# clvrai/mopa-rl

Hardware: AMD Instinct MI355X
Metric: valid-state collision checks/sec (higher is better)
Workload: dtype f64; 1 GPU; SawyerPushObstacle-v0 state validity (FK + collision), 4096 envs/GPU x 256 states/env per step, states 50% uniform joint-box samples + 50% near-init N(0,0.3); envs_per_gpu=4096, states_per_env=256, parallelism=env-shard x1

## Files before the change

include/mopa_hip.h:

```cpp
#ifndef MOPA_HIP_H
#define MOPA_HIP_H
#include <stdint.h>

#ifdef __cplusplus
extern "C" {
#endif

#define MOPA_OK 0
#define MOPA_ERR_INVALID_ARG 1
#define MOPA_ERR_UNSUPPORTED 2
#define MOPA_ERR_HIP 3
#define MOPA_ERR_LIMIT 4

#define MOPA_PLAN_OK 0
#define MOPA_PLAN_NO_EXACT (-4)
#define MOPA_PLAN_INVALID_GOAL (-5)

#define MOPA_FAR 1.0e10

enum { MOPA_GEOM_PLANE = 0, MOPA_GEOM_SPHERE = 2, MOPA_GEOM_CAPSULE = 3, MOPA_GEOM_CYLINDER = 5, MOPA_GEOM_BOX = 6, MOPA_GEOM_MESH = 7 };
enum { MOPA_JNT_FREE = 0, MOPA_JNT_BALL = 1, MOPA_JNT_SLIDE = 2, MOPA_JNT_HINGE = 3 };

typedef struct MopaModel {
    int32_t nq, nbody, njnt, ngeom, npair;
// ... 70 lines not shown
int mopa_glue_rows_batch(MopaScene *scene, double *path_dev , const int32_t *path_len_dev ,
                         const double *attached_dev , int64_t E, int32_t max_path, void *stream);
int mopa_scene_num_active(const MopaScene *scene);
int mopa_scene_active_idx(const MopaScene *scene, int32_t *out );
int mopa_scene_num_pairs(const MopaScene *scene);
int mopa_scene_lds_bytes(const MopaScene *scene);
int mopa_scene_valid_kernel(const MopaScene *scene, int64_t N, char *out, int32_t cap );
int mopa_scene_motion_kernel(const MopaScene *scene, int64_t N, char *out, int32_t cap );
int mopa_scene_k1_baked(const MopaScene *scene);
int mopa_scene_k1_export(const MopaSceneDesc *desc, int64_t *sizes , double *dbl, int32_t *ints, int32_t *tab, void *hdr,
                         uint64_t *fingerprint);
int mopa_scene_hdr_offset(const char *field);
int mopa_scene_k1_export_glued(const MopaSceneDesc *desc, int32_t body_a, int32_t body_b, int64_t *sizes , double *dbl, int32_t *ints,
                               int32_t *tab, void *hdr, uint64_t *fingerprint);
int mopa_k1_baked_fk_host(int index, int64_t n, const double *q_active, const double *qpos_env, double *out);

int mopa_is_valid_batch(MopaScene *scene, const double *q_active_dev , const double *qpos_env_dev ,
                        int64_t N, int64_t samples_per_env, uint8_t *valid_dev , double *min_dist_dev ,
                        void *stream);

int mopa_check_motion_batch(MopaScene *scene, const double *qa_dev , const double *qb_dev ,
                            const double *qpos_env_dev , int64_t N, int64_t samples_per_env,
                            uint8_t *valid_dev , void *stream);

int mopa_plan_batch(MopaScene *scene, const double *start_dev , const double *goal_dev , int64_t E,
                    const MopaPlanParams *params, double *path_dev , int32_t *path_len_dev ,
                    int32_t *status_dev , int64_t *n_checks_dev , void *stream);

int mopa_simplify_paths_batch(MopaScene *scene, int64_t E, int32_t max_path, double *path_dev ,
                              int32_t *path_len_dev , const int32_t *status_dev , uint64_t seed,
                              uint64_t env_id_base, const uint64_t *env_ids_dev , const uint64_t *seeds_dev ,
                              int32_t passes, int64_t *info_dev , void *stream);
int mopa_simplify_paths_max_path(const MopaScene *scene);

// ... 388 lines not shown
```

mopa_rl_amd/_lib.py:

```python
from __future__ import annotations

import ctypes as C
import os
from typing import Optional

import numpy as np

_HERE = os.path.dirname(os.path.abspath(__file__))
LIB_PATH = os.environ.get("MOPA_HIP_LIB", os.path.join(_HERE, "csrc", "libmopa_hip.so"))

MOPA_OK = 0
MOPA_FAR = 1.0e10
PLAN_OK, PLAN_NO_EXACT, PLAN_INVALID_GOAL = 0, -4, -5

_dp = C.POINTER(C.c_double)
_ip = C.POINTER(C.c_int32)

EXPORTED_SYMBOLS = [
    "mopa_last_error", "mopa_version", "mopa_device_count", "mopa_scene_create", "mopa_scene_destroy",
    "mopa_scene_create_glued", "mopa_scene_glue", "mopa_glue_attach_batch", "mopa_glue_rows_batch", "mopa_scene_k1_export_glued",
    "mopa_scene_num_active", "mopa_scene_active_idx", "mopa_scene_num_pairs", "mopa_scene_lds_bytes", "mopa_scene_valid_kernel",
    "mopa_scene_motion_kernel",
    "mopa_scene_k1_baked", "mopa_scene_k1_export", "mopa_scene_hdr_offset", "mopa_k1_baked_fk_host",
    "mopa_is_valid_batch", "mopa_check_motion_batch", "mopa_plan_batch", "mopa_simplify_paths_batch", "mopa_simplify_paths_max_path", "mopa_shortcut_paths_batch", "mopa_shortcut_paths_max_path", "mopa_smooth_paths_batch", "mopa_smooth_paths_max_path",
    "mopa_plan_star_batch", "mopa_plan_star", "mopa_plan_star_k", "mopa_star_params_size",
    "mopa_plan_race_batch", "mopa_plan_race", "mopa_race_params_size", "mopa_pullback_batch", "mopa_is_valid_state", "mopa_plan",
    "mopa_planner_status", "mopa_debug_fk", "mopa_debug_pair_dist", "mopa_contacts_batch", "mopa_contacts_state",
    "mopa_contact_frames_batch", "mopa_contact_frames_state", "mopa_geom_frames_batch", "mopa_geom_frames_host",
    "mopa_env_create", "mopa_env_destroy", "mopa_env_obs_dim", "mopa_env_action_dim", "mopa_env_step_batch", "mopa_env_exec_batch", "mopa_env_desired_batch",
    "mopa_env_attach_dynamics", "mopa_env_attach_contacts", "mopa_env_set_contact_stats", "mopa_rollout_stage", "mopa_rollout_pool_pick", "mopa_rollout_step_size", "mopa_reuse_batch", "mopa_replay_append", "mopa_replay_sample", "mopa_ct_desc_size", "mopa_env_contact_arena", "mopa_env_dyn_dofs", "mopa_env_dyn_qvel_width", "mopa_env_dyn_forward_batch", "mopa_env_dyn_substeps_batch", "mopa_env_step_dyn_batch",
    "mopa_pusher_dyn_desc_size", "mopa_env_attach_pusher_dynamics", "mopa_env_set_pusher_stats", "mopa_env_pusher_substeps_batch",
    "mopa_env_step_pusher_batch", "mopa_env_set_contact_force",
    "mopa_ik_create", "mopa_ik_destroy", "mopa_ik_solve_batch", "mopa_ik_site_pose_batch", "mopa_ik_targets_batch",
    "mopa_ik_targets_pos_batch", "mopa_ik_displacement_pos_batch",
    "mopa_paths_unwrap_batch", "mopa_paths_unwrap_seam_batch", "mopa_paths_walk_batch", "mopa_paths_assemble_batch", "mopa_interpolate_batch",
]


class MopaError(RuntimeError):
# ... 148 lines not shown
    L.mopa_version.restype = C.c_char_p
    L.mopa_device_count.restype = C.c_int
    L.mopa_scene_create.argtypes = [C.POINTER(MopaSceneDesc), C.POINTER(vp)]
    L.mopa_scene_destroy.argtypes = [vp]
    L.mopa_scene_destroy.restype = None
    L.mopa_scene_create_glued.argtypes = [C.POINTER(MopaSceneDesc), C.c_int32, C.c_int32, C.POINTER(vp)]
    L.mopa_scene_glue.argtypes = [vp, _ip]
    L.mopa_glue_attach_batch.argtypes = [vp, vp, C.c_int64, vp, vp]
    L.mopa_glue_rows_batch.argtypes = [vp, vp, vp, vp, C.c_int64, C.c_int32, vp]
    L.mopa_scene_k1_export_glued.argtypes = [vp, C.c_int32, C.c_int32, vp, vp, vp, vp, vp, vp]
    L.mopa_scene_num_active.argtypes = [vp]
    L.mopa_scene_active_idx.argtypes = [vp, _ip]
    L.mopa_scene_num_pairs.argtypes = [vp]
    L.mopa_scene_lds_bytes.argtypes = [vp]
    L.mopa_is_valid_batch.argtypes = [vp, vp, vp, C.c_int64, C.c_int64, vp, vp, vp]
    L.mopa_check_motion_batch.argtypes = [vp, vp, vp, vp, C.c_int64, C.c_int64, vp, vp]
    L.mopa_plan_batch.argtypes = [vp, vp, vp, C.c_int64, C.POINTER(MopaPlanParams), vp, vp, vp, vp, vp]
    L.mopa_simplify_paths_batch.argtypes = [vp, C.c_int64, C.c_int32, vp, vp, vp, C.c_uint64, C.c_uint64, vp, vp, C.c_int32, vp, vp]
    L.mopa_simplify_paths_max_path.argtypes = [vp]
    L.mopa_shortcut_paths_batch.argtypes = [vp, C.c_int64, C.c_int32, vp, vp, vp, C.c_uint64, C.c_uint64, vp, vp, C.c_int32, C.c_int32, vp, vp]
    L.mopa_shortcut_paths_max_path.argtypes = [vp]
    L.mopa_smooth_paths_batch.argtypes = [vp, C.c_int64, C.c_int32, vp, vp, vp, C.c_uint64, C.c_uint64, vp, vp, C.c_int32, C.c_int32, vp, vp]
    L.mopa_smooth_paths_max_path.argtypes = [vp]
    L.mopa_plan_star_batch.argtypes = [vp, vp, vp, C.c_int64, C.POINTER(MopaStarParams), vp, vp, vp, vp, vp, vp]
    L.mopa_plan_star.argtypes = [vp, _dp, _dp, C.POINTER(MopaStarParams), _dp, C.POINTER(C.c_int32), C.POINTER(C.c_int32),
                                 C.POINTER(C.c_double), C.POINTER(C.c_int64)]
    L.mopa_plan_star_k.argtypes = [C.c_int32, C.c_int64, C.c_double]
    L.mopa_star_params_size.argtypes = []
    L.mopa_plan_race_batch.argtypes = [vp, vp, vp, C.c_int64, C.POINTER(MopaRaceParams), vp, vp, vp, vp, vp, vp, vp, vp]
    L.mopa_plan_race.argtypes = [vp, _dp, _dp, C.POINTER(MopaRaceParams), _dp, C.POINTER(C.c_int32), C.POINTER(C.c_int32),
# ... 49 lines not shown
    L.mopa_ik_destroy.argtypes = [vp]
    L.mopa_ik_destroy.restype = None
    L.mopa_ik_solve_batch.argtypes = [vp, C.c_int64, vp, vp, vp, C.c_double, C.c_int32, C.c_double, C.c_double, C.c_double, C.c_double,
                                      vp, vp, vp, vp]
    L.mopa_ik_site_pose_batch.argtypes = [vp, C.c_int64, vp, vp, vp, vp]
    L.mopa_ik_targets_batch.argtypes = [vp, C.c_int64, vp, vp, vp, C.c_int64, C.c_double, C.POINTER(C.c_double), C.POINTER(C.c_double), vp, vp, vp]
    L.mopa_ik_targets_pos_batch.argtypes = [vp, C.c_int64, vp, vp, C.c_int64, C.c_int32, C.c_double, C.POINTER(C.c_double), C.POINTER(C.c_double), vp, vp]
    L.mopa_ik_displacement_pos_batch.argtypes = [vp, C.c_int64, vp, vp, C.c_int64, C.c_int32, C.c_double, C.POINTER(C.c_double), C.POINTER(C.c_double),
                                                 C.c_int32, C.c_double, C.c_double, C.c_double, C.c_double, vp, vp, vp, vp, vp, vp, vp]
    L.mopa_scene_valid_kernel.argtypes = [vp, C.c_int64, C.c_char_p, C.c_int32]
    L.mopa_scene_motion_kernel.argtypes = [vp, C.c_int64, C.c_char_p, C.c_int32]
    L.mopa_scene_k1_baked.argtypes = [vp]
    L.mopa_scene_k1_export.argtypes = [vp, vp, vp, vp, vp, vp, vp]
    L.mopa_scene_hdr_offset.argtypes = [C.c_char_p]
    L.mopa_k1_baked_fk_host.argtypes = [C.c_int, C.c_int64, vp, vp, vp]
    i32, i64, f64 = C.c_int32, C.c_int64, C.c_double
    L.mopa_paths_unwrap_batch.argtypes = [C.c_int, i64, i32, i32, vp, i32, vp, vp, vp, f64, i32, vp, vp, vp, vp, vp, vp, vp, vp]
    L.mopa_paths_unwrap_seam_batch.argtypes = [C.c_int, i64, i32, i32, vp, i32, vp, vp, vp, f64, i32, vp, vp, vp, vp, vp, vp, vp, C.c_uint64, vp]
    L.mopa_paths_walk_batch.argtypes = [C.c_int, i64, i32, i32, vp, i32, vp, vp, f64, vp, vp, vp, vp, vp, vp, vp, vp]
    L.mopa_paths_assemble_batch.argtypes = [C.c_int, i64, i32, vp, i32, vp, vp, vp, vp, vp, vp, vp, i32, vp, vp]
    L.mopa_interpolate_batch.argtypes = [vp, i64, i32, i32, vp, vp, f64, vp, vp, vp, vp, vp]
    _lib = L
    return L


def check(rc: int) -> None:
    if rc != MOPA_OK:
        raise MopaError(f"libmopa_hip error {rc}: {lib().mopa_last_error().decode()}")


# ... 344 lines not shown
```

mopa_rl_amd/batch.py:

```python
from __future__ import annotations

import ctypes as C
import os

import numpy as np
from typing import Optional, Tuple

from . import _lib


def _torch():
    import torch
    return torch


def _ptr(t) -> C.c_void_p:
    return C.c_void_p(t.data_ptr())


def _check_f64(t, name, cols=None):
    torch = _torch()
    if t.dtype != torch.float64 or not t.is_cuda or not t.is_contiguous():
        raise _lib.MopaError(f"{name} must be a contiguous float64 tensor on the GPU")
    if cols is not None and (t.dim() != 2 or t.shape[1] != cols):
# ... 99 lines not shown
    return (4 if path_shortcut else 0) | vertex


def k9_entry(vertex_simplify, path_shortcut, path_smooth) -> Optional[str]:
    return "smooth_paths" if path_smooth else "shortcut_paths" if path_shortcut else "simplify_paths" if vertex_simplify else None


class BatchPlanner:

    def __init__(self, scene: "_lib.Scene"):
        self.scene = scene
        self.na = scene.na
        self.nq = scene.nq

    def is_valid(self, q_active, qpos_env, samples_per_env: Optional[int] = None, want_min_dist: bool = False,
                 out=None, stream=None, guard: bool = False):
        torch = _torch()
        _check_f64(q_active, "q_active", self.na)
        _check_f64(qpos_env, "qpos_env", self.nq)
        N = q_active.shape[0]
        spe = int(samples_per_env) if samples_per_env is not None else max(1, N // max(1, qpos_env.shape[0]))
        if N and (N + spe - 1) // spe > qpos_env.shape[0]:
            raise _lib.MopaError("qpos_env has fewer rows than ceil(N / samples_per_env)")
        valid = out if out is not None else torch.empty(N, dtype=torch.uint8, device=q_active.device)
        md = torch.empty(N, dtype=torch.float64, device=q_active.device) if want_min_dist else None
        _lib.check(_lib.lib().mopa_is_valid_batch(self.scene.handle, _ptr(q_active), _ptr(qpos_env), N, spe, _ptr(valid),
                                                  _ptr(md) if md is not None else None, _stream_handle(stream)))
        if guard and self.scene.npair_pruned and N:
            sc = self.scene
            dev = q_active.device
            if getattr(self, "_guard_t", None) is None or self._guard_t[0].device != dev:
                pos = {int(a): k for k, a in enumerate(sc.active_idx)}
                act = [k for k, a in enumerate(sc.guard_adr) if int(a) in pos]
                pas = [k for k, a in enumerate(sc.guard_adr) if int(a) not in pos]
                mk = lambda a, dt: torch.as_tensor(np.asarray(a), dtype=dt, device=dev)
                self._guard_t = (mk([pos[int(sc.guard_adr[k])] for k in act], torch.long), mk(sc.guard_lo[act], torch.float64), mk(sc.guard_hi[act], torch.float64),
                                 mk(sc.guard_adr[pas], torch.long), mk(sc.guard_lo[pas], torch.float64), mk(sc.guard_hi[pas], torch.float64))
            ia, la, ha, ip_, lp, hp = self._guard_t
            qa = q_active[:, ia]
            oor = ((qa < la) | (qa > ha)).any(dim=1)
# ... 348 lines not shown
```

mopa_rl_amd/csrc/mopa_hip.hip:

```cpp
#include <hip/hip_runtime.h>

#include <algorithm>
#include <cmath>
#include <cstdio>
#include <cstdlib>
#include <cstddef>
#include <cstring>
#include <string>
#include <utility>
#include <vector>

#include <map>
#include <mutex>
#include "../../include/mopa_hip.h"
#include "mopa_device.hpp"
#include "mopa_frames.hpp"
#include "mopa_fk.hpp"
#include "mopa_host.hpp"

using namespace mopa;

static thread_local std::string g_err;
int mopa_fail(int code, const std::string &msg) {
    g_err = msg;
// ... 482 lines not shown
extern "C" int mopa_scene_k1_export_glued(const MopaSceneDesc *desc, int32_t body_a, int32_t body_b, int64_t *sizes, double *dbl, int32_t *ints,
                                          int32_t *tab, void *hdr, uint64_t *fingerprint) {
    if (body_a < 0 || body_b < 0) return fail(MOPA_ERR_INVALID_ARG, "glue: body id out of range");
    return scene_k1_export(desc, body_a, body_b, sizes, dbl, ints, tab, hdr, fingerprint);
}

extern "C" int mopa_scene_hdr_offset(const char *field) {
    if (!field) return -1;
#define MOPA_HDR_FIELD(f_) if (!std::strcmp(field, #f_)) return (int)offsetof(SceneHdr, f_);
    MOPA_HDR_FIELD(na) MOPA_HDR_FIELD(nq) MOPA_HDR_FIELD(n_pq) MOPA_HDR_FIELD(nmb) MOPA_HDR_FIELD(nmg) MOPA_HDR_FIELD(nsf)
    MOPA_HDR_FIELD(n_save) MOPA_HDR_FIELD(n_pas_b) MOPA_HDR_FIELD(n_dbl) MOPA_HDR_FIELD(n_int) MOPA_HDR_FIELD(o_mbr) MOPA_HDR_FIELD(o_mbd)
    MOPA_HDR_FIELD(o_mgd) MOPA_HDR_FIELD(o_sf_pos) MOPA_HDR_FIELD(o_sf_quat) MOPA_HDR_FIELD(o_sf_mat) MOPA_HDR_FIELD(o_act_ref)
    MOPA_HDR_FIELD(o_pq_adr) MOPA_HDR_FIELD(o_mg_geom) MOPA_HDR_FIELD(thr)
    MOPA_HDR_FIELD(o_mb_parent) MOPA_HDR_FIELD(o_chain_adr) MOPA_HDR_FIELD(o_chain_len) MOPA_HDR_FIELD(o_chain_items) MOPA_HDR_FIELD(o_g_mb)
    MOPA_HDR_FIELD(o_mb_load) MOPA_HDR_FIELD(o_mb_save) MOPA_HDR_FIELD(pfk_maxlen) MOPA_HDR_FIELD(n_gp) MOPA_HDR_FIELD(npair) MOPA_HDR_FIELD(o_pairs)
#undef MOPA_HDR_FIELD
    return -1;
}

namespace {
struct K1HostSink {
    double *out;
    void operator()(int m, V3 gp, Q4 gq) {
        double *o = out + 12 * m;
        o[0] = gp.x; o[1] = gp.y; o[2] = gp.z;
        quat2mat(o + 3, gq);
    }
};
template <class TR>
void k1_fk_host(int64_t n, const double *q_active, const double *qpos_env, double *out) {
    for (int64_t s = 0; s < n; s++) {
        K1HostSink sink{out + (size_t)s * 12 * TR::nmg};
        k1_fk_baked<TR>(q_active + (size_t)s * TR::na, qpos_env + (size_t)s * TR::nq, sink, std::make_integer_sequence<int, TR::nmb>{});
    }
}
}
extern "C" int mopa_k1_baked_fk_host(int index, int64_t n, const double *q_active, const double *qpos_env, double *out) {
    if (n < 0 || (n > 0 && (!q_active || !qpos_env || !out))) return fail(MOPA_ERR_INVALID_ARG, "null argument / negative count");
#define MOPA_K1_FK_HOST(i_, T_) if (index == i_) { k1_fk_host<T_>(n, q_active, qpos_env, out); return MOPA_OK; }
    MOPA_K1_BAKED_SCENES(MOPA_K1_FK_HOST)
#undef MOPA_K1_FK_HOST
    return fail(MOPA_ERR_INVALID_ARG, "no baked scene #" + std::to_string(index));
}

static int scene_create(const MopaSceneDesc *desc, int glue_a, int glue_b, MopaScene **out) {
    if (!desc || !out) return fail(MOPA_ERR_INVALID_ARG, "null argument");
    MopaScene *S = new MopaScene();
    {
        const int rc = scene_build_host(desc, S, glue_a, glue_b);
        if (rc != MOPA_OK) { delete S; return rc; }
    }
    {
        const char *eb = std::getenv("MOPA_K1_BAKED");
        const uint64_t fp = k1_fingerprint(S);
        const bool allowed = !(eb && std::string(eb) == "0") && S->k1.use_v5 && S->k1.v5_cen_lds && S->n_mesh_gp == 0 && S->glue_b < 0;
        S->k1_baked = allowed ? k1_baked_index(fp) : 0;
// ... 186 lines not shown
```

mopa_rl_amd/csrc/mopa_valid_launch.inc:

```

static int64_t k1_lane_min(const MopaScene *S) { return S->k1.v2_forced ? 64 : std::max<int64_t>(64, (int64_t)S->n_cu * 36); }
static int64_t k1_motion_expand_min(const MopaScene *S) { return S->k1.v2_forced ? 64 : std::max<int64_t>(64, (int64_t)S->n_cu * 16); }

using K1FnV1 = decltype(&k_is_valid<false, false>);
using K1FnV2 = decltype(&k_is_valid_v2<false, false>);
using K1FnV5 = decltype(&k_is_valid_v5<false, true, false>);
#define MOPA_K1_COUNT(i_, T_) +1
constexpr int kK1BakedScenes = 0 MOPA_K1_BAKED_SCENES(MOPA_K1_COUNT);
#undef MOPA_K1_COUNT

static K1FnV1 k1_kernel_v1(bool want_md, bool mesh) {
    static const K1FnV1 tab[2][2] = {{k_is_valid<false, false>, k_is_valid<true, false>}, {k_is_valid<false, true>, k_is_valid<true, true>}};
    return tab[mesh][want_md];
}
static K1FnV2 k1_kernel_v2(bool want_md, bool mesh) {
    static const K1FnV2 tab[2][2] = {{k_is_valid_v2<false, false>, k_is_valid_v2<true, false>}, {k_is_valid_v2<false, true>, k_is_valid_v2<true, true>}};
    return tab[mesh][want_md];
}
static K1FnV5 k1_kernel_v5(bool want_md, bool cen_lds, bool gate, int baked) {
    static const K1FnV5 generic[3][2] = {{k_is_valid_v5<false, true, false>, k_is_valid_v5<true, true, false>},
                                         {k_is_valid_v5<false, false, false>, k_is_valid_v5<true, false, false>},
                                         {k_is_valid_v5<false, false, true>, k_is_valid_v5<true, false, true>}};
    if (cen_lds && gate) return nullptr;
    if (!baked) return generic[cen_lds ? 0 : (gate ? 2 : 1)][want_md];
// ... 191 lines not shown
    {
        unsigned long long hp[6];
        (void)hipStreamSynchronize(st);
        (void)hipMemcpy(hp, d_prof, 48, hipMemcpyDeviceToHost);
        if (hp[5]) fprintf(stderr, "[v2 profile] per tile cycles: body %.0f geom %.0f cull+push %.0f flush %.0f total %.0f (tiles %llu)\n",
                           (double)hp[0] / hp[5], (double)hp[1] / hp[5], (double)hp[2] / hp[5], (double)hp[3] / hp[5], (double)hp[4] / hp[5], hp[5]);
    }
#endif
    return MOPA_OK;
}

extern "C" int mopa_is_valid_batch(MopaScene *S, const double *q_active, const double *qpos_env, int64_t N,
                                   int64_t samples_per_env, uint8_t *valid, double *min_dist, void *stream) {
    return launch_is_valid(S, q_active, qpos_env, N, samples_per_env, nullptr, valid, min_dist, stream, nullptr, true);
}
```

mopa_rl_amd/csrc/mopa_valid_v5.inc:

```

constexpr int kEntCapV5Max = 1024;
constexpr int kBatCapV5 = 128;
constexpr int kMprCapV5 = 128;
constexpr int kMprRow = 32;
constexpr float kCullEps = 2.0e-5f;

struct K1Generic {
    static constexpr bool kBaked = false;
};
#include "mopa_valid_v5_baked.inc"

template <class TR, int M, bool WANT_MD, int K>
MOPA_D void v5_cull_baked(float cx, float cy, float cz, const float *cen_lane, unsigned &surv_lo, unsigned &surv_hi,
                          unsigned long long &deep_mask, unsigned long long &any_kept) {
    constexpr int e = TR::padr[M] + K;
    constexpr float c0 = __builtin_bit_cast(float, TR::tab[8 * e + 0]), c1 = __builtin_bit_cast(float, TR::tab[8 * e + 1]);
    constexpr float c2 = __builtin_bit_cast(float, TR::tab[8 * e + 2]), c3 = __builtin_bit_cast(float, TR::tab[8 * e + 3]);
    constexpr float c4 = __builtin_bit_cast(float, TR::tab[8 * e + 4]), c5 = __builtin_bit_cast(float, TR::tab[8 * e + 5]);
    constexpr float c6 = __builtin_bit_cast(float, TR::tab[8 * e + 6]);
    bool keep;
    if constexpr (K < TR::nmov[M]) {
        const float *pc = cen_lane + ((TR::tab[8 * e + 7] >> 14) & 0xff) * 3 * 64;
        const float dx = cx - pc[0], dy = cy - pc[64], dz = cz - pc[128];
        const float d2 = fmaf(dz, dz, fmaf(dy, dy, dx * dx));
        if constexpr (!WANT_MD && TR::tab[8 * e + 0] != 0u) deep_mask |= __ballot(d2 < c0);
        keep = !(d2 > c3);
    } else if constexpr (K < TR::nmov[M] + TR::nstat[M]) {
        const float dx = cx - c0, dy = cy - c1, dz = cz - c2;
        keep = !((fmaf(dz, dz, fmaf(dy, dy, dx * dx)) > c3) | (fabsf(dx) > c4) | (fabsf(dy) > c5) | (fabsf(dz) > c6));
    } else {
        const float dx = cx - c0, dy = cy - c1, dz = cz - c2;
        keep = !(fmaf(dz, c6, fmaf(dy, c5, dx * c4)) > c3);
    }
    if constexpr (K < 32) surv_lo |= keep ? (1u << K) : 0u;
    else surv_hi |= keep ? (1u << (K - 32)) : 0u;
    any_kept |= __ballot(keep) ? (1ull << K) : 0ull;
}
template <class TR, int M, bool WANT_MD, int... K>
MOPA_D void v5_pass_a_baked(float cx, float cy, float cz, const float *cen_lane, unsigned &surv_lo, unsigned &surv_hi,
                            unsigned long long &deep_mask, unsigned long long &any_kept, std::integer_sequence<int, K...>) {
    (v5_cull_baked<TR, M, WANT_MD, K>(cx, cy, cz, cen_lane, surv_lo, surv_hi, deep_mask, any_kept), ...);
}
template <class TR, bool WANT_MD, int... M>
MOPA_D void v5_pass_a_dispatch(int m, float cx, float cy, float cz, const float *cen_lane, unsigned &surv_lo, unsigned &surv_hi,
                               unsigned long long &deep_mask, unsigned long long &any_kept, std::integer_sequence<int, M...>) {
    (void)((m == M ? (v5_pass_a_baked<TR, M, WANT_MD>(cx, cy, cz, cen_lane, surv_lo, surv_hi, deep_mask, any_kept,
                                                     std::make_integer_sequence<int, TR::pnum[M]>{}), true)
                   : false) || ...);
}

MOPA_HD constexpr double k1_bits(unsigned long long b) { return __builtin_bit_cast(double, b); }
template <class TR>
struct K1FkRegs {
    V3 pos;
    Q4 quat;
    double mat[9];
    V3 save_pos[TR::n_save];
    Q4 save_quat[TR::n_save];
};
template <class TR, int M, class Sink>
MOPA_HD void k1_fk_geom(const K1FkRegs<TR> &r, Sink &sink) {
    constexpr const unsigned long long *gd = TR::fk_gd[M];
    const V3 gp = add3(r.pos, mat_vec(r.mat, V3{k1_bits(gd[0]), k1_bits(gd[1]), k1_bits(gd[2])}));
    const Q4 gq = quat_mul(r.quat, Q4{k1_bits(gd[3]), k1_bits(gd[4]), k1_bits(gd[5]), k1_bits(gd[6])});
    sink(M, gp, gq);
}
template <class TR, int B, class Sink, int... G>
MOPA_HD void k1_fk_body(K1FkRegs<TR> &r, const double *qact, const double *sn, const double *cs, const double *pv, Sink &sink,
                        std::integer_sequence<int, G...>) {
    constexpr const int *bi = TR::fk_body[B];
    constexpr int load = bi[0], sf = bi[1], save = bi[2], mgadr = bi[3], jn = bi[5], jt = bi[6], src = bi[8];
    constexpr bool jp0 = bi[7] != 0;
    constexpr const unsigned long long *bd = TR::fk_bd[B];
    static_assert(jn <= 1 && sizeof...(G) == bi[4], "baked walk: one joint per body at most");
    if constexpr (jn == 1 && jt == J_FREE) {
        fk_free_step(pv + (src - TR::na), r.pos, r.quat);
    } else {
        V3 ppos;
        Q4 pquat;
        if constexpr (load == -2) {
// ... 18 lines not shown
            if constexpr (src < TR::na) apply_joint_sc(jt, ax, jp, jp0, qact[src] - ref, sn[src], cs[src], r.pos, r.quat);
            else apply_joint(jt, ax, jp, jp0, pv[src - TR::na] - ref, r.pos, r.quat);
        }
        r.quat = quat_normalize(r.quat);
    }
    quat2mat(r.mat, r.quat);
    if constexpr (save >= 0) {
        r.save_pos[save] = r.pos;
        r.save_quat[save] = r.quat;
    }
    (k1_fk_geom<TR, mgadr + G>(r, sink), ...);
}
template <class TR, class Sink, int... B>
MOPA_HD void k1_fk_baked(const double *qa_row, const double *env_row, Sink &sink, std::integer_sequence<int, B...>) {
    static_assert(TR::na <= 8 && TR::n_pq >= 1 && TR::n_save >= 1, "baked walk: at most 8 active values; array sizes padded to 1");
    double qact[TR::na], pv[TR::n_pq], sn[TR::na], cs[TR::na];
#pragma unroll
    for (int a = 0; a < TR::na; a++) qact[a] = qa_row[a];
#pragma unroll
    for (int k = 0; k < TR::n_pq; k++) pv[k] = env_row[TR::fk_pq_adr[k]];
#pragma unroll
    for (int a = 0; a < TR::na; a++) mopa_sincos(0.5 * (qact[a] - k1_bits(TR::fk_act_ref[a])), sn[a], cs[a]);
    K1FkRegs<TR> r;
    r.pos = V3{0.0, 0.0, 0.0};
    r.quat = Q4{1.0, 0.0, 0.0, 0.0};
    (k1_fk_body<TR, B>(r, qact, sn, cs, pv, sink, std::make_integer_sequence<int, TR::fk_body[B][4]>{}), ...);
}
struct V5FkSink {
    double *slab;
    float *cen;
    MOPA_D void operator()(int m, V3 gp, Q4 gq) {
        double *sp = slab + (size_t)m * kSlabStride;
        pose7_st<64>(sp, gp, gq);
        float *cp = cen + (size_t)m * 3 * 64;
        cp[0] = (float)gp.x; cp[64] = (float)gp.y; cp[128] = (float)gp.z;
    }
};

struct V5Lds {
    float *cen;
    unsigned *ent;
    unsigned *bat;
    unsigned *bat2;
    unsigned long long *bad;
    unsigned long long *md;
    bool tp;
};
MOPA_HD int v5_lds_per_wave(int nmg, int ent_cap, bool want_md) { return ((nmg * 3 * 64 * 4) + ent_cap * 4 + 2 * kBatCapV5 * 4 + (want_md ? 64 * 8 : 0) + 8 + 15) & ~15; }

MOPA_D void v5_load_rec2(double (&R1)[15], double (&R2)[15], const SceneHdr &h, const double *D, const double *slab_tile,
                         int gA, int movA, int slotA, int gB, int movB, int slotB, int slA, int slB) {
// ... 200 lines not shown
    const long long n_tiles = (N + 63) >> 6;
    for (;;) {
        long long tile = 0;
        if (lane == 0) tile = (long long)atomicAdd(tile_ctr, 1ull);
        tile = __shfl(tile, 0, 64);
        const bool fin = tile >= n_tiles;
        if (!fin) {
        long long s = tile * 64 + lane;
        const bool act = s < N;
        if (!act) s = N - 1;
        const double *qa_row = q_active + s * h.na;
        const double *env_row = qpos_env + (env_idx ? (long long)env_idx[s] : s / samples_per_env) * h.nq;
        if (lane == 0) *q.bad = 0ull;
        if (WANT_MD) q.md[lane] = f64_sortable(0.0);

#ifdef MOPA_V5_FK_REPS
        for (int fk_rep = 0; fk_rep < MOPA_V5_FK_REPS; fk_rep++)
#endif
        if constexpr (TR::kBaked) {
            double *fk_slab = slab;
            asm volatile("" : "+v"(fk_slab));
            V5FkSink sink{fk_slab, q.cen + lane};
            k1_fk_baked<TR>(qa_row, env_row, sink, std::make_integer_sequence<int, TR::nmb>{});
#ifdef MOPA_V5_FK_REPS
            asm volatile("" ::: "memory");
#endif
        } else {
            double *ps = reinterpret_cast<double *>(q.ent);
            bool tile_poses = false;
            if (!GATE && h.n_pas_b > 0) {
                const unsigned long long er = (unsigned long long)env_row;
                const unsigned long long e0 = ((unsigned long long)(unsigned)__builtin_amdgcn_readfirstlane((int)(er >> 32)) << 32) | (unsigned)__builtin_amdgcn_readfirstlane((int)(unsigned)er);
                tile_poses = __all(er == e0);
            }
            q.tp = !GATE && tile_poses;
            if (!GATE && tile_poses) {
                for (int lv = 0; lv < h.n_pas_lv; lv++) {
                    const int i = s_int[h.o_pas_lv + lv] + lane;
// ... 153 lines not shown
                for (int m = bi.mgadr; m < bi.mgadr + bi.mgnum; m++) {
                    const double *gd = s_dbl + h.o_mgd + 8 * m;
                    const V3 gp = add3(pos, mat_vec(mat, ld3(gd)));
                    const Q4 gq = quat_mul(quat, Q4{gd[3], gd[4], gd[5], gd[6]});
                    double *sp = slab + (size_t)m * kSlabStride;
                    pose7_st<64>(sp, gp, gq);
                    float *cp = CEN_LDS ? q.cen + (size_t)m * 3 * 64 + lane : gcen + (size_t)m * 3 * 64;
                    cp[0] = (float)gp.x; cp[64] = (float)gp.y; cp[128] = (float)gp.z;
                }
            }
        }
        wave_sync();

        bool dead = !act;
        bool need_mesh = false;
        int n_ent = 0;
        unsigned present = 0u;
        for (int m = 0; m < h.nmg; m++) {
            int p0, pn;
            if (GATE) {
                p0 = g_tab[8 * h.n_gp + h.nmg + 2 * m]; pn = g_tab[8 * h.n_gp + h.nmg + 2 * m + 1];
            } else {
                const V2GeomI gi = *reinterpret_cast<const V2GeomI *>(GI + h.o_mgr + 4 * m);
                p0 = gi.padr; pn = gi.pnum;
            }
            if (pn == 0) continue;
            float cx, cy, cz;
            if (CEN_LDS) {
                const float *cp = q.cen + (size_t)m * 3 * 64 + lane;
                cx = cp[0]; cy = cp[64]; cz = cp[128];
// ... 217 lines not shown
```

mopa_rl_amd/csrc/mopa_valid_v5_baked.inc:

```

struct K1Baked_SawyerPushObstacle {
    static constexpr bool kBaked = true;
    static constexpr unsigned long long kFingerprint = 0x85dfbe79baeda04bull;
    static constexpr int nmg = 14;
    static constexpr int padr[nmg] = {0, 1, 3, 4, 5, 10, 15, 29, 47, 65, 83, 101, 119, 138};
    static constexpr int pnum[nmg] = {1, 2, 1, 1, 5, 5, 14, 18, 18, 18, 18, 18, 19, 17};
    static constexpr int nmov[nmg] = {0, 0, 0, 0, 1, 1, 3, 5, 5, 5, 5, 5, 6, 13};
    static constexpr int nstat[nmg] = {0, 1, 0, 0, 3, 3, 10, 12, 12, 12, 12, 12, 12, 3};
    static constexpr int npl[nmg] = {1, 1, 1, 1, 1, 1, 1, 1, 1, 1, 1, 1, 1, 1};
    static constexpr unsigned tab[1240] = {
        0x00000000u, 0x00000000u, 0x00000000u, 0x3d8f66a5u, 0x00000000u, 0x00000000u, 0x3f800000u, 0x40001000u,
        0x00000000u, 0x00000000u, 0x3f88f5c3u, 0x3dd74fecu, 0x3e852158u, 0x3e852158u, 0x3e999c39u, 0x00000603u,
        0x00000000u, 0x00000000u, 0x00000000u, 0x3e38572au, 0x00000000u, 0x00000000u, 0x3f800000u, 0x40001000u,
        0x00000000u, 0x00000000u, 0x00000000u, 0x3e0e4865u, 0x00000000u, 0x00000000u, 0x3f800000u, 0x40001300u,
        0x00000000u, 0x00000000u, 0x00000000u, 0x3d8f66a5u, 0x00000000u, 0x00000000u, 0x3f800000u, 0x40001000u,
        0x3d67a9acu, 0x00000000u, 0x00000000u, 0x3e2c26b4u, 0x00000000u, 0x00000000u, 0x00000000u, 0x00007505u,
        0xbea66666u, 0x00000000u, 0x3f11eb85u, 0x3eac19a5u, 0x3eae171au, 0x3edc2b95u, 0x3efd7344u, 0x00000901u,
        0xbca3d70au, 0x00000000u, 0x3f28f5c3u, 0x3eb150c3u, 0x3ed1ee24u, 0x3ed1ee24u, 0x3f0a3ec0u, 0x00000b02u,
        0x00000000u, 0x00000000u, 0x3f88f5c3u, 0x3e0f6b23u, 0x3e9ebaf1u, 0x3e9ebaf1u, 0x3eb335d2u, 0x00000b03u,
        0x00000000u, 0x00000000u, 0x00000000u, 0x3e6b8a5du, 0x00000000u, 0x00000000u, 0x3f800000u, 0x40001100u,
        0x3d5e062au, 0x00000000u, 0x00000000u, 0x3db2405bu, 0x00000000u, 0x00000000u, 0x00000000u, 0x00007505u,
        0xbea66666u, 0x00000000u, 0x3f11eb85u, 0x3e5d3203u, 0x3e666ba4u, 0x3ea14a4du, 0x3ec291fcu, 0x00000901u,
        0xbca3d70au, 0x00000000u, 0x3f28f5c3u, 0x3e65928au, 0x3e970cddu, 0x3e970cddu, 0x3ed99c39u, 0x00000b02u,
        0x00000000u, 0x00000000u, 0x3f88f5c3u, 0x3d89a388u, 0x3e47b352u, 0x3e47b352u, 0x3e70a915u, 0x00000b03u,
// ... 182 lines not shown
        {0x0000000000000000ull, 0x0000000000000000ull, 0x3fbc28f5c28f5c29ull, 0x3ff0000000000000ull, 0x0000000000000000ull, 0x0000000000000000ull, 0x0000000000000000ull},
        {0x0000000000000000ull, 0x0000000000000000ull, 0x3fa999999999999aull, 0x3ff0000000000000ull, 0x0000000000000000ull, 0x0000000000000000ull, 0x0000000000000000ull},
        {0x0000000000000000ull, 0x3f8eb851eb851eb8ull, 0xbf847ae147ae147bull, 0x3ff0000000000000ull, 0x0000000000000000ull, 0x0000000000000000ull, 0x0000000000000000ull},
        {0x0000000000000000ull, 0x0000000000000000ull, 0x0000000000000000ull, 0x3ff0000000000000ull, 0x0000000000000000ull, 0x0000000000000000ull, 0x0000000000000000ull},
        {0xbf989374bc6a7efaull, 0x0000000000000000ull, 0x0000000000000000ull, 0x3fe6a2ecb934b59aull, 0x0000000000000000ull, 0x3fe69e4fd79ac743ull, 0x0000000000000000ull},
        {0x0000000000000000ull, 0x0000000000000000ull, 0x0000000000000000ull, 0x3ff0000000000000ull, 0x0000000000000000ull, 0x0000000000000000ull, 0x0000000000000000ull},
        {0x0000000000000000ull, 0xbfa47ae147ae147bull, 0x0000000000000000ull, 0x3ff0000000000000ull, 0x0000000000000000ull, 0x0000000000000000ull, 0x0000000000000000ull},
        {0x0000000000000000ull, 0x0000000000000000ull, 0x0000000000000000ull, 0x3ff0000000000000ull, 0x0000000000000000ull, 0x0000000000000000ull, 0x0000000000000000ull},
    };
    static constexpr unsigned long long fk_sf[nsf][16] = {
        {0x0000000000000000ull, 0x0000000000000000ull, 0x0000000000000000ull, 0x3ff0000000000000ull, 0x0000000000000000ull, 0x0000000000000000ull, 0x0000000000000000ull, 0x3ff0000000000000ull, 0x0000000000000000ull, 0x0000000000000000ull, 0x0000000000000000ull, 0x3ff0000000000000ull, 0x0000000000000000ull, 0x0000000000000000ull, 0x0000000000000000ull, 0x3ff0000000000000ull},
        {0x0000000000000000ull, 0x0000000000000000ull, 0x3fee666666666666ull, 0x3ff0000000000000ull, 0x0000000000000000ull, 0x0000000000000000ull, 0x0000000000000000ull, 0x3ff0000000000000ull, 0x0000000000000000ull, 0x0000000000000000ull, 0x0000000000000000ull, 0x3ff0000000000000ull, 0x0000000000000000ull, 0x0000000000000000ull, 0x0000000000000000ull, 0x3ff0000000000000ull},
    };
    static constexpr unsigned long long fk_act_ref[na] = {0x0000000000000000ull, 0x0000000000000000ull, 0x0000000000000000ull, 0x0000000000000000ull, 0x0000000000000000ull, 0x0000000000000000ull, 0x0000000000000000ull};
    static constexpr int fk_pq_adr[n_pq] = {7, 8, 27, 28, 29, 30, 31, 32, 33};
};

#define MOPA_K1_BAKED_SCENES(X) X(1, K1Baked_SawyerPushObstacle)
```

Before: 2.286 billion checks/s.

## Evaluate a resident collision pair inside baked FK and skip it in culling

Adds a 'resident' pair mechanism. One statically known geom pair (sphere-capsule) has its exact distance computed inside the baked FK walk, while both geom poses are still in registers. That pair is then removed from the cull and pair-distance passes. The idea is to save the slab round-trip and cull work for a pair that nearly always needs an exact check. It costs extra registers in FK and an unconditional f64 distance per state. It also adds a counted is_valid entry point that reads N from the device, and a host reference for the resident distances.

```diff
diff --git a/include/mopa_hip.h b/include/mopa_hip.h
--- a/include/mopa_hip.h
+++ b/include/mopa_hip.h
@@ -108,10 +108,14 @@
 int mopa_scene_k1_export_glued(const MopaSceneDesc *desc, int32_t body_a, int32_t body_b, int64_t *sizes , double *dbl, int32_t *ints,
                                int32_t *tab, void *hdr, uint64_t *fingerprint);
 int mopa_k1_baked_fk_host(int index, int64_t n, const double *q_active, const double *qpos_env, double *out);
+int mopa_k1_baked_resident_host(int index, int64_t n, const double *q_active, const double *qpos_env, double *out, int32_t *n_res);
 
 int mopa_is_valid_batch(MopaScene *scene, const double *q_active_dev , const double *qpos_env_dev ,
                         int64_t N, int64_t samples_per_env, uint8_t *valid_dev , double *min_dist_dev ,
                         void *stream);
+int mopa_is_valid_batch_counted(MopaScene *scene, const double *q_active_dev , const double *qpos_env_dev ,
+                                int64_t N, int64_t samples_per_env, uint8_t *valid_dev , double *min_dist_dev ,
+                                const int64_t *n_dev, void *stream);
 
 int mopa_check_motion_batch(MopaScene *scene, const double *qa_dev , const double *qb_dev ,
                             const double *qpos_env_dev , int64_t N, int64_t samples_per_env,
diff --git a/mopa_rl_amd/_lib.py b/mopa_rl_amd/_lib.py
--- a/mopa_rl_amd/_lib.py
+++ b/mopa_rl_amd/_lib.py
@@ -21,8 +21,8 @@
     "mopa_scene_create_glued", "mopa_scene_glue", "mopa_glue_attach_batch", "mopa_glue_rows_batch", "mopa_scene_k1_export_glued",
     "mopa_scene_num_active", "mopa_scene_active_idx", "mopa_scene_num_pairs", "mopa_scene_lds_bytes", "mopa_scene_valid_kernel",
     "mopa_scene_motion_kernel",
-    "mopa_scene_k1_baked", "mopa_scene_k1_export", "mopa_scene_hdr_offset", "mopa_k1_baked_fk_host",
-    "mopa_is_valid_batch", "mopa_check_motion_batch", "mopa_plan_batch", "mopa_simplify_paths_batch", "mopa_simplify_paths_max_path", "mopa_shortcut_paths_batch", "mopa_shortcut_paths_max_path", "mopa_smooth_paths_batch", "mopa_smooth_paths_max_path",
+    "mopa_scene_k1_baked", "mopa_scene_k1_export", "mopa_scene_hdr_offset", "mopa_k1_baked_fk_host", "mopa_k1_baked_resident_host",
+    "mopa_is_valid_batch", "mopa_is_valid_batch_counted", "mopa_check_motion_batch", "mopa_plan_batch", "mopa_simplify_paths_batch", "mopa_simplify_paths_max_path", "mopa_shortcut_paths_batch", "mopa_shortcut_paths_max_path", "mopa_smooth_paths_batch", "mopa_smooth_paths_max_path",
     "mopa_plan_star_batch", "mopa_plan_star", "mopa_plan_star_k", "mopa_star_params_size",
     "mopa_plan_race_batch", "mopa_plan_race", "mopa_race_params_size", "mopa_pullback_batch", "mopa_is_valid_state", "mopa_plan",
     "mopa_planner_status", "mopa_debug_fk", "mopa_debug_pair_dist", "mopa_contacts_batch", "mopa_contacts_state",
@@ -201,6 +201,7 @@
     L.mopa_scene_num_pairs.argtypes = [vp]
     L.mopa_scene_lds_bytes.argtypes = [vp]
     L.mopa_is_valid_batch.argtypes = [vp, vp, vp, C.c_int64, C.c_int64, vp, vp, vp]
+    L.mopa_is_valid_batch_counted.argtypes = [vp, vp, vp, C.c_int64, C.c_int64, vp, vp, vp, vp]
     L.mopa_check_motion_batch.argtypes = [vp, vp, vp, vp, C.c_int64, C.c_int64, vp, vp]
     L.mopa_plan_batch.argtypes = [vp, vp, vp, C.c_int64, C.POINTER(MopaPlanParams), vp, vp, vp, vp, vp]
     L.mopa_simplify_paths_batch.argtypes = [vp, C.c_int64, C.c_int32, vp, vp, vp, C.c_uint64, C.c_uint64, vp, vp, C.c_int32, vp, vp]
@@ -280,6 +281,7 @@
     L.mopa_scene_k1_export.argtypes = [vp, vp, vp, vp, vp, vp, vp]
     L.mopa_scene_hdr_offset.argtypes = [C.c_char_p]
     L.mopa_k1_baked_fk_host.argtypes = [C.c_int, C.c_int64, vp, vp, vp]
+    L.mopa_k1_baked_resident_host.argtypes = [C.c_int, C.c_int64, vp, vp, vp, vp]
     i32, i64, f64 = C.c_int32, C.c_int64, C.c_double
     L.mopa_paths_unwrap_batch.argtypes = [C.c_int, i64, i32, i32, vp, i32, vp, vp, vp, f64, i32, vp, vp, vp, vp, vp, vp, vp, vp]
     L.mopa_paths_unwrap_seam_batch.argtypes = [C.c_int, i64, i32, i32, vp, i32, vp, vp, vp, f64, i32, vp, vp, vp, vp, vp, vp, vp, C.c_uint64, vp]
diff --git a/mopa_rl_amd/batch.py b/mopa_rl_amd/batch.py
--- a/mopa_rl_amd/batch.py
+++ b/mopa_rl_amd/batch.py
@@ -137,7 +137,7 @@
         self.nq = scene.nq
 
     def is_valid(self, q_active, qpos_env, samples_per_env: Optional[int] = None, want_min_dist: bool = False,
-                 out=None, stream=None, guard: bool = False):
+                 out=None, stream=None, guard: bool = False, n_dev=None):
         torch = _torch()
         _check_f64(q_active, "q_active", self.na)
         _check_f64(qpos_env, "qpos_env", self.nq)
@@ -147,6 +147,12 @@
             raise _lib.MopaError("qpos_env has fewer rows than ceil(N / samples_per_env)")
         valid = out if out is not None else torch.empty(N, dtype=torch.uint8, device=q_active.device)
         md = torch.empty(N, dtype=torch.float64, device=q_active.device) if want_min_dist else None
+        if n_dev is not None:
+            if guard or n_dev.dtype != torch.int64 or n_dev.numel() != 1 or n_dev.device != q_active.device:
+                raise _lib.MopaError("n_dev: one int64 on the states' device, without guard")
+            _lib.check(_lib.lib().mopa_is_valid_batch_counted(self.scene.handle, _ptr(q_active), _ptr(qpos_env), N, spe, _ptr(valid),
+                                                              _ptr(md) if md is not None else None, _ptr(n_dev), _stream_handle(stream)))
+            return (valid, md) if want_min_dist else valid
         _lib.check(_lib.lib().mopa_is_valid_batch(self.scene.handle, _ptr(q_active), _ptr(qpos_env), N, spe, _ptr(valid),
                                                   _ptr(md) if md is not None else None, _stream_handle(stream)))
         if guard and self.scene.npair_pruned and N:
diff --git a/mopa_rl_amd/csrc/mopa_hip.hip b/mopa_rl_amd/csrc/mopa_hip.hip
--- a/mopa_rl_amd/csrc/mopa_hip.hip
+++ b/mopa_rl_amd/csrc/mopa_hip.hip
@@ -520,6 +520,7 @@
     MOPA_HDR_FIELD(o_pq_adr) MOPA_HDR_FIELD(o_mg_geom) MOPA_HDR_FIELD(thr)
     MOPA_HDR_FIELD(o_mb_parent) MOPA_HDR_FIELD(o_chain_adr) MOPA_HDR_FIELD(o_chain_len) MOPA_HDR_FIELD(o_chain_items) MOPA_HDR_FIELD(o_g_mb)
     MOPA_HDR_FIELD(o_mb_load) MOPA_HDR_FIELD(o_mb_save) MOPA_HDR_FIELD(pfk_maxlen) MOPA_HDR_FIELD(n_gp) MOPA_HDR_FIELD(npair) MOPA_HDR_FIELD(o_pairs)
+    MOPA_HDR_FIELD(o_g_rec) MOPA_HDR_FIELD(o_g_type)
 #undef MOPA_HDR_FIELD
     return -1;
 }
@@ -532,6 +533,12 @@
         o[0] = gp.x; o[1] = gp.y; o[2] = gp.z;
         quat2mat(o + 3, gq);
     }
+    void resident(int, double) {}
+};
+struct K1ResHostSink {
+    double *out;
+    void operator()(int, V3, Q4) {}
+    void resident(int r, double d) { out[r] = d; }
 };
 template <class TR>
 void k1_fk_host(int64_t n, const double *q_active, const double *qpos_env, double *out) {
@@ -540,12 +547,26 @@
         k1_fk_baked<TR>(q_active + (size_t)s * TR::na, qpos_env + (size_t)s * TR::nq, sink, std::make_integer_sequence<int, TR::nmb>{});
     }
 }
+template <class TR>
+void k1_res_host(int64_t n, const double *q_active, const double *qpos_env, double *out) {
+    for (int64_t s = 0; s < n; s++) {
+        K1ResHostSink sink{out + (size_t)s * k1_n_res<TR>};
+        k1_fk_baked<TR>(q_active + (size_t)s * TR::na, qpos_env + (size_t)s * TR::nq, sink, std::make_integer_sequence<int, TR::nmb>{});
+    }
+}
 }
 extern "C" int mopa_k1_baked_fk_host(int index, int64_t n, const double *q_active, const double *qpos_env, double *out) {
     if (n < 0 || (n > 0 && (!q_active || !qpos_env || !out))) return fail(MOPA_ERR_INVALID_ARG, "null argument / negative count");
 #define MOPA_K1_FK_HOST(i_, T_) if (index == i_) { k1_fk_host<T_>(n, q_active, qpos_env, out); return MOPA_OK; }
     MOPA_K1_BAKED_SCENES(MOPA_K1_FK_HOST)
 #undef MOPA_K1_FK_HOST
+    return fail(MOPA_ERR_INVALID_ARG, "no baked scene #" + std::to_string(index));
+}
+extern "C" int mopa_k1_baked_resident_host(int index, int64_t n, const double *q_active, const double *qpos_env, double *out, int32_t *n_res) {
+    if (n < 0 || (n > 0 && (!q_active || !qpos_env || !out))) return fail(MOPA_ERR_INVALID_ARG, "null argument / negative count");
+#define MOPA_K1_RES_HOST(i_, T_) if (index == i_) { if (n_res) *n_res = k1_n_res<T_>; if (k1_n_res<T_> > 0) k1_res_host<T_>(n, q_active, qpos_env, out); return MOPA_OK; }
+    MOPA_K1_BAKED_SCENES(MOPA_K1_RES_HOST)
+#undef MOPA_K1_RES_HOST
     return fail(MOPA_ERR_INVALID_ARG, "no baked scene #" + std::to_string(index));
 }
 
diff --git a/mopa_rl_amd/csrc/mopa_valid_launch.inc b/mopa_rl_amd/csrc/mopa_valid_launch.inc
--- a/mopa_rl_amd/csrc/mopa_valid_launch.inc
+++ b/mopa_rl_amd/csrc/mopa_valid_launch.inc
@@ -229,3 +229,8 @@
                                    int64_t samples_per_env, uint8_t *valid, double *min_dist, void *stream) {
     return launch_is_valid(S, q_active, qpos_env, N, samples_per_env, nullptr, valid, min_dist, stream, nullptr, true);
 }
+extern "C" int mopa_is_valid_batch_counted(MopaScene *S, const double *q_active, const double *qpos_env, int64_t N, int64_t samples_per_env,
+                                           uint8_t *valid, double *min_dist, const int64_t *n_dev, void *stream) {
+    if (!n_dev) return fail(MOPA_ERR_INVALID_ARG, "null argument");
+    return launch_is_valid(S, q_active, qpos_env, N, samples_per_env, nullptr, valid, min_dist, stream, reinterpret_cast<const long long *>(n_dev), true);
+}
diff --git a/mopa_rl_amd/csrc/mopa_valid_v5.inc b/mopa_rl_amd/csrc/mopa_valid_v5.inc
--- a/mopa_rl_amd/csrc/mopa_valid_v5.inc
+++ b/mopa_rl_amd/csrc/mopa_valid_v5.inc
@@ -10,9 +10,23 @@
 };
 #include "mopa_valid_v5_baked.inc"
 
+constexpr int kResMax = 2;
+#ifdef MOPA_V5_NO_RESIDENT
+template <class TR> constexpr int k1_n_res = 0;
+#else
+template <class TR> constexpr int k1_n_res = TR::n_res;
+#endif
+template <class TR>
+MOPA_HD constexpr bool k1_is_resident(int M, int K) {
+    for (int r = 0; r < k1_n_res<TR>; r++)
+        if (TR::res[r][0] == M && TR::res[r][1] == K) return true;
+    return false;
+}
+
 template <class TR, int M, bool WANT_MD, int K>
 MOPA_D void v5_cull_baked(float cx, float cy, float cz, const float *cen_lane, unsigned &surv_lo, unsigned &surv_hi,
                           unsigned long long &deep_mask, unsigned long long &any_kept) {
+    if constexpr (!k1_is_resident<TR>(M, K)) {
     constexpr int e = TR::padr[M] + K;
     constexpr float c0 = __builtin_bit_cast(float, TR::tab[8 * e + 0]), c1 = __builtin_bit_cast(float, TR::tab[8 * e + 1]);
     constexpr float c2 = __builtin_bit_cast(float, TR::tab[8 * e + 2]), c3 = __builtin_bit_cast(float, TR::tab[8 * e + 3]);
@@ -35,6 +49,7 @@
     if constexpr (K < 32) surv_lo |= keep ? (1u << K) : 0u;
     else surv_hi |= keep ? (1u << (K - 32)) : 0u;
     any_kept |= __ballot(keep) ? (1ull << K) : 0ull;
+    }
 }
 template <class TR, int M, bool WANT_MD, int... K>
 MOPA_D void v5_pass_a_baked(float cx, float cy, float cz, const float *cen_lane, unsigned &surv_lo, unsigned &surv_hi,
@@ -57,13 +72,48 @@
     double mat[9];
     V3 save_pos[TR::n_save];
     Q4 save_quat[TR::n_save];
+    V3 res_pos[kResMax];
+    Q4 res_quat[kResMax];
 };
+template <int TYPE>
+MOPA_HD void k1_res_rec(double (&R)[15], const V3 &p, const Q4 &q, const unsigned long long *size) {
+    R[GO_POS] = p.x; R[GO_POS + 1] = p.y; R[GO_POS + 2] = p.z;
+    if constexpr (TYPE != G_SPHERE) {
+        quat2mat(R + GO_MAT, q);
+    } else {
+#pragma unroll
+        for (int i = 0; i < 9; i++) R[GO_MAT + i] = 0.0;
+    }
+    R[GO_SIZE] = k1_bits(size[0]); R[GO_SIZE + 1] = k1_bits(size[1]); R[GO_SIZE + 2] = k1_bits(size[2]);
+}
+template <class TR, int M, int R, class Sink>
+MOPA_HD void k1_fk_resident(K1FkRegs<TR> &r, const V3 &gp, const Q4 &gq, Sink &sink) {
+    constexpr int sa = TR::res[R][2], sb = TR::res[R][3], code = TR::res[R][4], ta = TR::res[R][5], tb = TR::res[R][6];
+    static_assert(sa != sb && ta <= tb && (code == PC_SPHERE_SPHERE || code == PC_SPHERE_CAPSULE || code == PC_CAPSULE_CAPSULE),
+                  "resident pair: two geoms in routine order, closed-form class");
+    constexpr bool a_first = sa < sb;
+    if constexpr (M == (a_first ? sa : sb)) {
+        r.res_pos[R] = gp;
+        if constexpr ((a_first ? ta : tb) != G_SPHERE) r.res_quat[R] = gq;
+        else r.res_quat[R] = Q4{1.0, 0.0, 0.0, 0.0};
+    } else if constexpr (M == (a_first ? sb : sa)) {
+        double R1[15], R2[15];
+        k1_res_rec<ta>(R1, a_first ? r.res_pos[R] : gp, a_first ? r.res_quat[R] : gq, TR::res_size[R]);
+        k1_res_rec<tb>(R2, a_first ? gp : r.res_pos[R], a_first ? gq : r.res_quat[R], TR::res_size[R] + 3);
+        sink.resident(R, geom_dist<false>(code, R1, ta, R2, tb));
+    }
+}
+template <class TR, int M, class Sink, int... R>
+MOPA_HD void k1_fk_residents(K1FkRegs<TR> &r, const V3 &gp, const Q4 &gq, Sink &sink, std::integer_sequence<int, R...>) {
+    (k1_fk_resident<TR, M, R>(r, gp, gq, sink), ...);
+}
 template <class TR, int M, class Sink>
-MOPA_HD void k1_fk_geom(const K1FkRegs<TR> &r, Sink &sink) {
+MOPA_HD void k1_fk_geom(K1FkRegs<TR> &r, Sink &sink) {
     constexpr const unsigned long long *gd = TR::fk_gd[M];
     const V3 gp = add3(r.pos, mat_vec(r.mat, V3{k1_bits(gd[0]), k1_bits(gd[1]), k1_bits(gd[2])}));
     const Q4 gq = quat_mul(r.quat, Q4{k1_bits(gd[3]), k1_bits(gd[4]), k1_bits(gd[5]), k1_bits(gd[6])});
     sink(M, gp, gq);
+    k1_fk_residents<TR, M>(r, gp, gq, sink, std::make_integer_sequence<int, k1_n_res<TR>>{});
 }
 template <class TR, int B, class Sink, int... G>
 MOPA_HD void k1_fk_body(K1FkRegs<TR> &r, const double *qact, const double *sn, const double *cs, const double *pv, Sink &sink,
@@ -112,6 +162,7 @@
 template <class TR, class Sink, int... B>
 MOPA_HD void k1_fk_baked(const double *qa_row, const double *env_row, Sink &sink, std::integer_sequence<int, B...>) {
     static_assert(TR::na <= 8 && TR::n_pq >= 1 && TR::n_save >= 1, "baked walk: at most 8 active values; array sizes padded to 1");
+    static_assert(TR::n_res <= kResMax, "baked walk: at most kResMax resident pairs");
     double qact[TR::na], pv[TR::n_pq], sn[TR::na], cs[TR::na];
 #pragma unroll
     for (int a = 0; a < TR::na; a++) qact[a] = qa_row[a];
@@ -133,6 +184,8 @@
         float *cp = cen + (size_t)m * 3 * 64;
         cp[0] = (float)gp.x; cp[64] = (float)gp.y; cp[128] = (float)gp.z;
     }
+    double res_d[kResMax];
+    MOPA_D void resident(int r, double d) { res_d[r] = d; }
 };
 
 struct V5Lds {
@@ -363,14 +416,17 @@
         if (lane == 0) *q.bad = 0ull;
         if (WANT_MD) q.md[lane] = f64_sortable(0.0);
 
+        double res_d[kResMax] = {};
 #ifdef MOPA_V5_FK_REPS
         for (int fk_rep = 0; fk_rep < MOPA_V5_FK_REPS; fk_rep++)
 #endif
         if constexpr (TR::kBaked) {
             double *fk_slab = slab;
             asm volatile("" : "+v"(fk_slab));
-            V5FkSink sink{fk_slab, q.cen + lane};
+            V5FkSink sink{fk_slab, q.cen + lane, {}};
             k1_fk_baked<TR>(qa_row, env_row, sink, std::make_integer_sequence<int, TR::nmb>{});
+#pragma unroll
+            for (int r = 0; r < kResMax; r++) res_d[r] = sink.res_d[r];
 #ifdef MOPA_V5_FK_REPS
             asm volatile("" ::: "memory");
 #endif
@@ -554,6 +610,23 @@
 
         bool dead = !act;
         bool need_mesh = false;
+        if constexpr (TR::kBaked) {
+            if constexpr (k1_n_res<TR> > 0) {
+                bool rbad = false;
+                unsigned long long rmd = f64_sortable(0.0);
+#pragma unroll
+                for (int r = 0; r < k1_n_res<TR>; r++) {
+                    rbad = rbad || (res_d[r] <= h.thr);
+                    const unsigned long long im = f64_sortable(res_d[r]);
+                    rmd = im < rmd ? im : rmd;
+                }
+                rbad = rbad && act;
+                const unsigned long long rmask = __ballot(rbad);
+                if (lane == 0 && rmask) *q.bad |= rmask;
+                if (WANT_MD) q.md[lane] = rmd;
+                else dead = dead || rbad;
+            }
+        }
         int n_ent = 0;
         unsigned present = 0u;
         for (int m = 0; m < h.nmg; m++) {
diff --git a/mopa_rl_amd/csrc/mopa_valid_v5_baked.inc b/mopa_rl_amd/csrc/mopa_valid_v5_baked.inc
--- a/mopa_rl_amd/csrc/mopa_valid_v5_baked.inc
+++ b/mopa_rl_amd/csrc/mopa_valid_v5_baked.inc
@@ -220,6 +220,9 @@
     };
     static constexpr unsigned long long fk_act_ref[na] = {0x0000000000000000ull, 0x0000000000000000ull, 0x0000000000000000ull, 0x0000000000000000ull, 0x0000000000000000ull, 0x0000000000000000ull, 0x0000000000000000ull};
     static constexpr int fk_pq_adr[n_pq] = {7, 8, 27, 28, 29, 30, 31, 32, 33};
+    static constexpr int n_res = 1;
+    static constexpr int res[1][7] = {{4, 0, 1, 4, 5, 2, 3}};
+    static constexpr unsigned long long res_size[1][6] = {{0x3fc70a3d70a3d70aull, 0x0000000000000000ull, 0x0000000000000000ull, 0x3faeb851eb851eb8ull, 0x3fc5c28f5c28f5c3ull, 0x0000000000000000ull}};
 };
 
 #define MOPA_K1_BAKED_SCENES(X) X(1, K1Baked_SawyerPushObstacle)
```

Result: faster. 2.336 billion checks/s (median of 6 runs) (+2.2%).
